# YuePanEdward/MULLS

Measured on NVIDIA H100. Metric: scan-pair registrations/sec (120k-pt 64-beam), higher is better.
Workload: dtype f32 geometry / f64 accumulation

## Files before the change

mulls_b200/csrc/device_types.cuh:

```cuda
#pragma once
#include <cstdint>
#include <cuda_runtime.h>

#include "../../include/mulls_b200/abi.h"
#include "search_core.cuh"

namespace mulls {

constexpr int kNumClasses = MULLS_NUM_CLASSES;
constexpr int kNumSegs = 2 * kNumClasses;
constexpr int kIterBlock = 128;
constexpr int kIngestBlock = 256;
constexpr int kTerms = 28;
constexpr int kMaxLevels = 12;
constexpr int kCoordBits = 12;
constexpr int kDedupMinSrc = 500;
constexpr unsigned kClaimFree = 0x7f7f7f7fu;
constexpr int kIterFlags = MULLS_MAX_TRACE_ITERS;

enum PairStatus : int { kRunning = 0, kNeedPosterior = 1, kDone = 2 };

struct ChunkDesc {
    uint32_t pair;
    uint32_t seg;
    uint32_t first;
};

struct PairConst {
    int max_iter;
    int used[kNumClasses];
    int w_balance, w_residual, w_dist, w_intensity;
    float z_xy_ratio;
    float win_pt2pt, win_pt2pl, win_pt2li;
    float thre_unit, thre_min, thre_rate;
    float conv_t, conv_r;
// ... 54 lines not shown
    int bb_src[6];
    int bb_tgt[6];
    uint64_t alg_bytes;
    int kl_keep[kNumSegs];
    uint32_t kl_rank[kNumSegs];
    uint64_t kl_prefix[kNumSegs];
    uint32_t kl_hist[kNumSegs][256];
};

struct LoopCtl {
    int it;
    int n_it_chunks;
    int n_pairs;
    int trace_on;
    int max_iter;
    unsigned solved;
    unsigned n_live[2];
    unsigned work[4];
};

struct DeviceArrays {
    const float4 *in_aos;
    uint64_t *keys_a, *keys_b;
    uint32_t *vals_a, *vals_b;
    float4 *tgt_pos, *tgt_nrm;
    float4 *src_pos[2], *src_nrm[2];
    int *src_prevj[2];
    float4 *src_cert[2];
    int *nn_idx;
    float *nn_d2;
    uint8_t *flags;
    int *corr_j;
    float *corr_w;
    unsigned *claim;
    HashEntry *hash;
    uint32_t hash_pool_entries;
    uint32_t *hash_used;
    uint32_t *blk_kept;
    double *partials;
    double *post_partials;
    PairConst *pc;
    PairState *ps;
    ChunkDesc *in_chunks;
    ChunkDesc *it_chunks;
    mulls_icp_trace *trace;
    int *xch_i32;
    double *xch_f64;
// ... 10 lines not shown
```

mulls_b200/csrc/kernels_ingest.cuh:

```cuda
#pragma once
#include "device_math.cuh"
#include "device_types.cuh"

namespace mulls {

template <bool kUndistort, bool kNormals>
__device__ __forceinline__ void load_input_point(const PairConst &pc, uint32_t seg, uint32_t local, float4 &pos, float4 &nrm) {
    const bool is_src = seg >= kNumClasses;
    const int cls = seg % kNumClasses;
    const bool undistort = kUndistort && is_src && pc.undistort && cls != MULLS_VERTEX;
    float x, y, z, intensity = 0.0f, curvature = 0.0f;
    float nx = 0.0f, ny = 0.0f, nz = 0.0f;
    const uint32_t fmt = pc.in_fmt[seg];
    if (fmt == 0u) {
        const float4 *in = pc.in_ptr[seg] + 3 * (size_t)local;
        const float4 a = in[0];
        x = a.x, y = a.y, z = a.z;
        if (kNormals) {
            const float4 b = in[1];
            const float4 c = in[2];
            nx = b.x, ny = b.y, nz = b.z;
            intensity = c.x, curvature = c.y;
        } else if (undistort) {
            curvature = reinterpret_cast<const float *>(in + 2)[1];
// ... 139 lines not shown
    for (int i = 0; i < 16; ++i) {
        ps.T_total[i] = pc.init[i];
        ps.T_inc[i] = (i % 5 == 0) ? 1.0 : 0.0;
    }
    for (int i = 0; i < 36; ++i) ps.cofactor[i] = ps.info[i] = (i % 7 == 0) ? 1.0 : 0.0;
    for (int i = 0; i < 6; ++i) ps.x[i] = 0.0;
    ps.sigma2 = 1.0;
    ps.thre = pc.thre_unit;
    ps.confidence = 1.0f;
    ps.status = kRunning;
    ps.code = 0;
    ps.iter = 0;
    ps.iters_entered = 0;
    ps.final_buf = 0;
    ps.alg_bytes = 0;
    if (pc.max_iter <= 0) {
        ps.status = kDone;
        const int left = atomicSub(A.running, 1) - 1;
        *A.h_running = left;
        __threadfence_system();
    }
}

template <bool kUndistort, bool kFiniteOnly = false>
__global__ void __launch_bounds__(kIngestBlock) k_make_keys(DeviceArrays A) {
    const ChunkDesc cd = A.in_chunks[blockIdx.x];
    const PairConst &pc = A.pc[cd.pair];
    PairState &ps = A.ps[cd.pair];
    const uint32_t seg = cd.seg;
    const uint32_t local = cd.first + threadIdx.x;
    const bool valid = local < pc.in_n[seg];
    bool inside = false;
    if (valid) {
        const size_t gi = (size_t)pc.in_off[seg] + local;
        float4 p, unused;
        load_input_point<kUndistort, false>(pc, seg, local, p, unused);
        const double *b = ps.ibb;
        inside = (double)p.x > b[0] && (double)p.x < b[3] && (double)p.y > b[1] && (double)p.y < b[4] &&
                 (double)p.z > b[2] && (double)p.z < b[5];
        if (kFiniteOnly) inside = inside && finite_xyz(p);
        uint64_t key = ~0ull;
        if (inside) {
            const int hi = (1 << kCoordBits) - 1;
            int cx = (int)floorf((p.x - ps.origin[0]) * ps.inv_h0);
            int cy = (int)floorf((p.y - ps.origin[1]) * ps.inv_h0);
            int cz = (int)floorf((p.z - ps.origin[2]) * ps.inv_h0);
            cx = min(max(cx, 0), hi);
            cy = min(max(cy, 0), hi);
            cz = min(max(cz, 0), hi);
            key = ((uint64_t)(cd.pair * kNumSegs + seg) << 36) | morton36((uint32_t)cx, (uint32_t)cy, (uint32_t)cz);
        }
        A.keys_a[gi] = key;
        A.vals_a[gi] = (uint32_t)gi;
    }
    const unsigned ballot = __ballot_sync(0xffffffffu, inside);
    if ((threadIdx.x & 31) == 0 && ballot) atomicAdd(&ps.seg_count[seg], (unsigned)__popc(ballot));
}

__device__ __forceinline__ uint64_t sample_key(uint32_t seed, uint32_t cloud_id, uint32_t index) {
    uint64_t z = (((uint64_t)seed << 40) ^ ((uint64_t)cloud_id << 32) ^ (uint64_t)index) + 0x9e3779b97f4a7c15ull;
    z = (z ^ (z >> 30)) * 0xbf58476d1ce4e5b9ull;
    z = (z ^ (z >> 27)) * 0x94d049bb133111ebull;
    return z ^ (z >> 31);
}

__global__ void k_keepless_plan(DeviceArrays A, int n_pairs) {
    const int p = blockIdx.x * blockDim.x + threadIdx.x;
    if (p >= n_pairs) return;
    const PairConst &pc = A.pc[p];
    PairState &ps = A.ps[p];
    for (int s = 0; s < kNumSegs; ++s) {
        ps.kl_keep[s] = -1;
        ps.kl_prefix[s] = 0;
        ps.kl_rank[s] = 0;
        for (int b = 0; b < 256; ++b) ps.kl_hist[s][b] = 0;
    }
    if (!pc.keep_less) return;
    const int S = kNumClasses;
    auto plan = [&](int seg, int keep) {
// ... 42 lines not shown
    PairState &ps = A.ps[p];
    for (int s = 0; s < kNumSegs; ++s) {
        if (ps.kl_keep[s] <= 0) continue;
        uint32_t cum = 0, rank = ps.kl_rank[s];
        int d = 0;
        for (; d < 256; ++d) {
            const uint32_t h = ps.kl_hist[s][d];
            if (cum + h >= rank) break;
            cum += h;
        }
        ps.kl_prefix[s] |= (uint64_t)d << (56 - 8 * pass);
        ps.kl_rank[s] = rank - cum;
        for (int b = 0; b < 256; ++b) ps.kl_hist[s][b] = 0;
    }
}

__global__ void __launch_bounds__(kIngestBlock) k_keepless_mark(DeviceArrays A) {
    const ChunkDesc cd = A.in_chunks[blockIdx.x];
    const PairConst &pc = A.pc[cd.pair];
    PairState &ps = A.ps[cd.pair];
    const uint32_t seg = cd.seg;
    const int keep = ps.kl_keep[seg];
    if (keep < 0) return;
    const uint32_t local = cd.first + threadIdx.x;
    bool drop = false;
    if (local < pc.in_n[seg]) {
        const size_t gi = (size_t)pc.in_off[seg] + local;
        if (A.keys_a[gi] != ~0ull) {
            drop = (keep == 0) || sample_key(pc.random_seed, seg, local) > ps.kl_prefix[seg];
            if (drop) A.keys_a[gi] = ~0ull;
        }
    }
    const unsigned b = __ballot_sync(0xffffffffu, drop);
    if ((threadIdx.x & 31) == 0 && b) atomicSub(&ps.seg_count[seg], (unsigned)__popc(b));
}

__global__ void k_seg_offsets(DeviceArrays A, int n_pairs) {
    __shared__ uint32_t carry;
    __shared__ uint32_t warp_sums[32];
    if (threadIdx.x == 0) carry = 0;
    __syncthreads();
    const int total = n_pairs * kNumSegs;
    for (int base = 0; base < total; base += blockDim.x) {
        const int i = base + threadIdx.x;
        uint32_t v = 0;
        if (i < total) v = A.ps[i / kNumSegs].seg_count[i % kNumSegs];
        uint32_t incl = v;
        for (int o = 1; o < 32; o <<= 1) {
            uint32_t t = __shfl_up_sync(0xffffffffu, incl, o);
            if ((threadIdx.x & 31) >= o) incl += t;
        }
        if ((threadIdx.x & 31) == 31) warp_sums[threadIdx.x >> 5] = incl;
        __syncthreads();
        if (threadIdx.x < 32) {
            uint32_t w = (threadIdx.x < (blockDim.x >> 5)) ? warp_sums[threadIdx.x] : 0;
            uint32_t wi = w;
            for (int o = 1; o < 32; o <<= 1) {
// ... 17 lines not shown
            ps.n_src[c] = (int)ps.seg_count[kNumClasses + c];
            ps.n_src_g[c] = ps.n_src[c];
            ps.n_corr[c] = 0;
            ps.n_corr_last[c] = 0;
        }
        int cnt = 0;
        if (pc.used[MULLS_PILLAR]) cnt += ps.n_src[MULLS_PILLAR];
        if (pc.used[MULLS_FACADE]) cnt += ps.n_src[MULLS_FACADE];
        if (pc.used[MULLS_BEAM]) cnt += ps.n_src[MULLS_BEAM];
        ps.source_feature_points_count = cnt;
    }
}

__device__ __forceinline__ int cell_top(const uint64_t *keys, uint32_t i, uint64_t kcur) {
    if (kcur == ~0ull || ((uint32_t)(kcur >> 36) % kNumSegs) >= kNumClasses) return -1;
    if (i == 0) return kMaxLevels - 1;
    const uint64_t kprev = keys[i - 1];
    if ((kprev >> 36) != (kcur >> 36)) return kMaxLevels - 1;
    const uint64_t diff = (kcur ^ kprev) & ((1ull << 36) - 1);
    if (diff == 0) return -1;
    return (63 - __clzll((long long)diff)) / 3;
}

template <bool kUndistort>
__global__ void __launch_bounds__(256) k_gather(DeviceArrays A, const uint64_t *keys, const uint32_t *vals, uint32_t n_total) {
    const uint32_t i = blockIdx.x * blockDim.x + threadIdx.x;
    const uint64_t key = i < n_total ? keys[i] : ~0ull;
    const uint32_t sg = (uint32_t)(key >> 36);
    const uint32_t pair = sg / kNumSegs, seg = sg % kNumSegs;
    const int top = cell_top(keys, i, key);
    const int cnt = top < 0 ? 0 : min(top, A.ps[pair].n_levels - 1) + 1;
    const bool is_tgt = key != ~0ull && seg < kNumClasses;
    const unsigned grp = __match_any_sync(0xffffffffu, is_tgt ? sg : 0xffffffffu);
    if (grp == 0xffffffffu) {
        const int tot = __reduce_add_sync(0xffffffffu, cnt);
        if ((threadIdx.x & 31) == 0 && tot > 0) atomicAdd(&A.ps[pair].hash_entries[seg], (unsigned)tot);
    } else if (cnt > 0) {
        atomicAdd(&A.ps[pair].hash_entries[seg], (unsigned)cnt);
    }
    if (key == ~0ull) return;
    const PairConst &pc = A.pc[pair];
    float4 pos, nrm;
    load_input_point<kUndistort, true>(pc, seg, vals[i] - pc.in_off[seg], pos, nrm);
    const uint32_t local = i - A.ps[pair].seg_start[seg];
    if (seg < kNumClasses) {
        const uint32_t d = pc.tgt_base[seg] + local;
        A.tgt_pos[d] = pos;
        A.tgt_nrm[d] = nrm;
    } else {
        const uint32_t d = pc.src_base[seg - kNumClasses] + local;
        if (pc.sharded) nrm.w = __int_as_float(__float_as_int(nrm.w) + (int)pc.src_index_base[seg - kNumClasses]);
        A.src_pos[0][d] = pos;
        A.src_nrm[0][d] = nrm;
    }
}

__device__ __forceinline__ void hash_insert(HashEntry *table, uint32_t hmask, uint32_t klo, uint32_t khi, uint32_t children,
                                            uint32_t start, uint32_t count) {
    uint32_t slot = cell_hash(klo, khi) & hmask;
    const unsigned long long packed = (unsigned long long)klo | ((unsigned long long)(khi | (children << 16)) << 32);
    while (true) {
        unsigned long long *kp = reinterpret_cast<unsigned long long *>(&table[slot]);
        if (atomicCAS(kp, 0ull, packed) == 0ull) {
            *reinterpret_cast<uint2 *>(&table[slot].start) = make_uint2(start, count);
            return;
        }
        slot = (slot + 1) & hmask;
    }
}

__device__ __forceinline__ uint32_t cell_end(const uint64_t *keys, uint32_t b, uint32_t hi, uint64_t p, int shift) {
    uint32_t in = b, out = hi, step = 1;
    while (in + step < hi) {
        if ((keys[in + step] >> shift) != p) {
            out = in + step;
            break;
        }
// ... 100 lines not shown
```

mulls_b200/csrc/mulls_b200.cu:

```cuda
#include <algorithm>
#include <atomic>
#include <cassert>
#include <memory>
#include <cmath>
#include <cstdio>
#include <chrono>
#include <cstring>
#include <string>
#include <vector>

#include <cub/device/device_radix_sort.cuh>
#include <cub/device/device_run_length_encode.cuh>
#include <cub/device/device_scan.cuh>
#include <cub/device/device_select.cuh>
#include <thrust/iterator/counting_iterator.h>

#include <dlfcn.h>
#include <mutex>

#include "device_types.cuh"
#include "host_pack.h"
#include "scan_io.h"
#include "kernels_ingest.cuh"
#include "kernels_iterate.cuh"
// ... 53 lines not shown
    return nccl_api().all_reduce(buf, buf, count, dtype == 0 ? 8 : 2, op == 0 ? 0 : 3, user, (cudaStream_t)stream);
}
}


struct mulls_map;

struct Scratch {
    void *p = nullptr;
    size_t bytes = 0;
    Scratch() = default;
    Scratch(const Scratch &) = delete;
    Scratch &operator=(const Scratch &) = delete;
    ~Scratch() { release(); }
    void release() {
        if (p) cudaFree(p);
        p = nullptr, bytes = 0;
    }
};

struct mulls_ctx {
    int device = 0;
    size_t max_pairs = 0, max_src = 0, max_tgt = 0;
    size_t cap_src = 0, cap_tgt = 0, cap_in = 0, cap_it_chunks = 0, cap_in_chunks = 0;
    cudaStream_t stream = nullptr;
    DeviceArrays A{};
    void *cub_temp = nullptr;
    size_t cub_temp_bytes = 0;
    mulls_icp_result *d_results = nullptr;
    mulls_icp_result *h_results = nullptr;
    uint32_t *h_flags = nullptr;
    int *h_running = nullptr;
    std::vector<cudaEvent_t> ev_done;
    mulls_icp_trace *d_trace = nullptr;
    std::vector<PairConst> h_pc;
    std::vector<ChunkDesc> h_in_chunks, h_it_chunks;
    size_t n_pairs = 0, n_in = 0, n_src_total = 0, n_tgt_total = 0;
    int max_iter_max = 0;
    bool uploaded = false;
    void *nccl_comm = nullptr;
    bool any_keep_less = false;
    bool grid_valid = false;
    int use_graph = 1;
    cudaGraph_t graph = nullptr;
    cudaGraphExec_t graph_exec = nullptr;
    int graph_key[2] = {-1, -1};
    uint64_t graph_body_launches = 0, graph_tail_launches = 0;
    LoopCtl *h_ctl = nullptr;
    int num_sms = 132;
    bool any_normal_shooting = false;
    bool any_undistort = false;
    int host_pack = 2;
    float4 *h_stage = nullptr;
    size_t h_stage_slots = 0;
    cudaEvent_t ev_begin = nullptr, ev_ingest = nullptr, ev_iter = nullptr, ev_end = nullptr, ev_h2d0 = nullptr;
    bool h2d_timed = false;
    float up_ms_pack = 0.f, up_ms_host = 0.f;
    std::vector<cudaEvent_t> ev_search;
    mulls_run_stats stats{};
// ... 163 lines not shown
    }
    mulls_ctx *ctx = new mulls_ctx();
    ctx->device = device;
    ctx->max_pairs = max_pairs;
    ctx->max_src = max_src_pts;
    ctx->max_tgt = max_tgt_pts;
    auto fail = [&](const char *what, cudaError_t err) -> mulls_ctx * {
        g_create_error = std::string("mulls_create: ") + what + ": " + cudaGetErrorString(err);
        mulls_destroy(ctx);
        return nullptr;
    };
    if ((e = cudaSetDevice(device)) != cudaSuccess) return fail("cudaSetDevice", e);
    if ((e = cudaStreamCreateWithFlags(&ctx->stream, cudaStreamNonBlocking)) != cudaSuccess) return fail("stream", e);
    const size_t cs = ctx->cap_src = max_pairs * max_src_pts;
    const size_t ct = ctx->cap_tgt = max_pairs * max_tgt_pts;
    const size_t cin = ctx->cap_in = cs + ct;
    if (cin >= (1ull << 31)) {
        g_create_error = "mulls_create: more than 2^31 points per context";
        mulls_destroy(ctx);
        return nullptr;
    }
    ctx->cap_it_chunks = ceil_div(cs, kIterBlock) + max_pairs * (kNumClasses + 1);
    ctx->cap_in_chunks = ceil_div(cin, kIngestBlock) + max_pairs * kNumSegs;
    DeviceArrays &A = ctx->A;
    float4 *in = nullptr;
#define ALLOC(ptr, n)                                                   \
    if ((e = dev_alloc(ctx, &(ptr), (n))) != cudaSuccess) return fail(#ptr, e)
    ALLOC(in, 3 * cin);
    A.in_aos = in;
    ALLOC(A.keys_a, cin);
    ALLOC(A.keys_b, cin);
    ALLOC(A.vals_a, cin);
    ALLOC(A.vals_b, cin);
    ALLOC(A.tgt_pos, ct + kScanOverrun);
    ALLOC(A.tgt_nrm, ct);
    for (int b = 0; b < 2; ++b) {
        ALLOC(A.src_pos[b], cs);
        ALLOC(A.src_nrm[b], cs);
        ALLOC(A.src_prevj[b], cs);
        ALLOC(A.src_cert[b], cs);
    }
    ALLOC(A.nn_idx, cs);
    ALLOC(A.nn_d2, cs);
    ALLOC(A.flags, cs);
    ALLOC(A.corr_j, cs);
    ALLOC(A.corr_w, cs);
    ALLOC(A.claim, ct);
    {
        size_t pool = 12 * ct + 64 * max_pairs * kNumClasses;
        if (pool >= (1ull << 32)) pool = (1ull << 32) - 1;
        A.hash_pool_entries = (uint32_t)pool;
        ALLOC(A.hash, pool);
    }
    ALLOC(A.hash_used, 3);
    ALLOC(A.ctl, 1);
    ALLOC(A.blk_kept, ctx->cap_it_chunks);
// ... 13 lines not shown
    ALLOC(ctx->d_results, max_pairs + ceil_div(max_pairs * sizeof(uint64_t), sizeof(mulls_icp_result)) + 1);
    ALLOC(ctx->d_trace, max_pairs);
    ALLOC(A.running, 1);
    ALLOC(A.xch_i32, 32);
    ALLOC(A.xch_f64, kNumClasses * kTerms + 8);
#undef ALLOC
    if ((e = cudaHostAlloc((void **)&ctx->h_running, (1 + kIterFlags) * sizeof(int), cudaHostAllocMapped)) != cudaSuccess)
        return fail("mapped flag", e);
    {
        int *dptr = nullptr;
        if ((e = cudaHostGetDevicePointer((void **)&dptr, ctx->h_running, 0)) != cudaSuccess) return fail("mapped flag", e);
        A.h_running = dptr;
        A.h_running_iter = dptr + 1;
    }
    ctx->ev_done.resize(MULLS_MAX_TRACE_ITERS);
    for (auto &ev : ctx->ev_done) cudaEventCreateWithFlags(&ev, cudaEventDisableTiming);
    A.trace = ctx->d_trace;
    if ((e = cudaMallocHost((void **)&ctx->h_results, max_pairs * (sizeof(mulls_icp_result) + sizeof(uint64_t)))) != cudaSuccess)
        return fail("pinned results", e);
    if ((e = cudaMallocHost((void **)&ctx->h_flags, 4 * sizeof(uint32_t))) != cudaSuccess) return fail("pinned flags", e);
    if ((e = cudaMallocHost((void **)&ctx->h_ctl, sizeof(LoopCtl))) != cudaSuccess) return fail("pinned control block", e);
    {
        size_t bytes = 0;
        cub::DeviceRadixSort::SortPairs(nullptr, bytes, A.keys_a, A.keys_b, A.vals_a, A.vals_b, (int)cin, 0, 64,
                                        ctx->stream);
        ctx->cub_temp_bytes = bytes;
        if ((e = cudaMalloc(&ctx->cub_temp, std::max<size_t>(bytes, 16))) != cudaSuccess) return fail("cub temp", e);
    }
    cudaEventCreate(&ctx->ev_begin);
    cudaEventCreate(&ctx->ev_ingest);
    cudaEventCreate(&ctx->ev_iter);
    cudaEventCreate(&ctx->ev_end);
    cudaEventCreate(&ctx->ev_h2d0);
    ctx->ev_search.resize(2 * MULLS_MAX_TRACE_ITERS);
    for (auto &ev : ctx->ev_search) cudaEventCreate(&ev);
    if ((e = cudaMemsetAsync(A.ps, 0, max_pairs * sizeof(PairState), ctx->stream)) != cudaSuccess) return fail("memset", e);
    if ((e = cudaStreamSynchronize(ctx->stream)) != cudaSuccess) return fail("sync", e);
    return ctx;
}

int mulls_set_tunable(mulls_ctx *ctx, const char *name, int value) {
    if (!ctx || !name) return MULLS_E_ARG;
    if (ctx->twin) {
        const int rc = mulls_set_tunable(ctx->twin, name, value);
        if (rc != MULLS_OK) return rc;
    }
    std::string n(name);
    if (n == "use_graph") ctx->use_graph = value;
    else if (n == "host_pack") ctx->host_pack = value;
    else if (n == "pack_threads") PackPool::get().ensure_workers(value);
    else return MULLS_E_ARG;
    return MULLS_OK;
}

int mulls_pack_rows(const float *aos48, size_t n, int format, float *out) {
    if ((n > 0 && (!aos48 || !out)) || (format != kFmtPacked28 && format != kFmtPacked32) || ((uintptr_t)out % 16) != 0)
        return MULLS_E_ARG;
    pack_rows(aos48, 0, n, format, out, out + 4 * n);
    _mm_sfence();
// ... 134 lines not shown
    for (int i = 0; i < 16; ++i) pc.init[i] = init[i];
    for (int i = 0; i < 6; ++i) pc.tbound[i] = P.target_bound[i];
    return MULLS_OK;
}

static int upload_impl(mulls_ctx *ctx, size_t n_pairs, const mulls_cloud_view *tgt, const mulls_cloud_view *src,
                       const mulls_icp_params *params, const double *init_guess, const uint32_t *src_index_base,
                       const uint32_t *src_global_n, bool resident = true, bool tgt_on_device = false) {
    if (!ctx || !tgt || !src || !params || !init_guess || n_pairs == 0) return MULLS_E_ARG;
    ctx->tree_map = nullptr;
    ctx->grid_valid = false;
    if (n_pairs > ctx->max_pairs) {
        ctx->err = "more pairs than the context was created for";
        return MULLS_E_CAPACITY;
    }
    CK(cudaSetDevice(ctx->device));
    ctx->uploaded = false;
    const double t_up0 = wall_ms();
    ctx->h2d_timed = false;
    ctx->up_ms_pack = 0.f;
    ctx->h_pc.assign(n_pairs, PairConst());
    ctx->h_in_chunks.clear();
    ctx->h_it_chunks.clear();
    size_t in_off = 0, s_off = 0, t_off = 0;
    int max_iter_max = 0;
    bool any_keep_less = false, any_shoot = false, any_undistort = false;
    for (size_t p = 0; p < n_pairs; ++p) {
        PairConst &pc = ctx->h_pc[p];
        int rc = build_pair_const(ctx, params[p], init_guess + 16 * p, pc);
        if (rc != MULLS_OK) return rc;
        max_iter_max = std::max(max_iter_max, pc.max_iter);
        any_keep_less = any_keep_less || pc.keep_less;
        any_shoot = any_shoot || pc.normal_shooting;
        any_undistort = any_undistort || pc.undistort;
        size_t ns = 0, nt = 0;
        for (int c = 0; c < kNumClasses; ++c) {
            nt += tgt[p * kNumClasses + c].n;
            ns += src[p * kNumClasses + c].n;
        }
        if (ns > ctx->max_src || nt > ctx->max_tgt) {
            ctx->err = "pair exceeds max_src_pts / max_tgt_pts of the context";
            return MULLS_E_CAPACITY;
        }
        for (int s = 0; s < kNumSegs; ++s) {
            const mulls_cloud_view &v = (s < kNumClasses) ? tgt[p * kNumClasses + s] : src[p * kNumClasses + (s - kNumClasses)];
            if (v.n > 0 && !v.aos48) return MULLS_E_ARG;
            pc.in_off[s] = (uint32_t)in_off;
            pc.in_n[s] = (uint32_t)v.n;
            for (size_t f = 0; f < v.n; f += kIngestBlock)
                ctx->h_in_chunks.push_back(ChunkDesc{(uint32_t)p, (uint32_t)s, (uint32_t)f});
            in_off += v.n;
        }
        pc.chunk_begin = (uint32_t)ctx->h_it_chunks.size();
        for (int c = 0; c < kNumClasses; ++c) {
            pc.tgt_base[c] = (uint32_t)t_off;
            pc.src_base[c] = (uint32_t)s_off;
            t_off += tgt[p * kNumClasses + c].n;
            const size_t n = src[p * kNumClasses + c].n;
            s_off += n;
            pc.class_chunk_begin[c] = (uint32_t)ctx->h_it_chunks.size();
            const size_t n_eff = (c == 0 && n == 0) ? 1 : n;
            for (size_t f = 0; f < n_eff; f += kIterBlock) ctx->h_it_chunks.push_back(ChunkDesc{(uint32_t)p, (uint32_t)c, (uint32_t)f});
            pc.src_index_base[c] = src_index_base ? src_index_base[c] : 0;
            pc.src_global_n[c] = src_global_n ? src_global_n[c] : (uint32_t)n;
        }
        pc.class_chunk_begin[kNumClasses] = (uint32_t)ctx->h_it_chunks.size();
        pc.chunk_end = (uint32_t)ctx->h_it_chunks.size();
        pc.sharded = src_index_base ? 1 : 0;
    }
    if (ctx->h_in_chunks.size() > ctx->cap_in_chunks || ctx->h_it_chunks.size() > ctx->cap_it_chunks) {
        ctx->err = "internal: chunk table capacity";
        return MULLS_E_CAPACITY;
    }
    size_t host_points = 0;
    for (size_t p = 0; p < n_pairs; ++p)
        for (int s = 0; s < kNumSegs; ++s)
            if (!(tgt_on_device && s < kNumClasses)) host_points += ctx->h_pc[p].in_n[s];
    const size_t kPackMinPoints = 1u << 18;
    bool tables_sent = false;
    const bool pack = ctx->host_pack == 1 || (ctx->host_pack == 2 && host_points >= kPackMinPoints);
    if (pack) {
        if (!ctx->h_stage) {
            const size_t slots = 2 * ctx->cap_in + 4 * kNumSegs * ctx->max_pairs;
            CK(cudaHostAlloc((void **)&ctx->h_stage, slots * sizeof(float4), cudaHostAllocDefault));
            ctx->h_stage_slots = slots;
        }
        CK(cudaStreamSynchronize(ctx->stream));
        PackPool &pool = PackPool::get();
        pool.ensure_workers(0);
        std::unique_ptr<std::atomic<int>[]> pending(new std::atomic<int>[n_pairs]);
        std::vector<size_t> slot_begin(n_pairs + 1, 0);
        std::vector<PackJob> jobs;
        const size_t kJobPts = 16384;
// ... 16 lines not shown
                float *pos = reinterpret_cast<float *>(ctx->h_stage + slot);
                float *nrm = reinterpret_cast<float *>(ctx->h_stage + slot + v.n);
                for (size_t f = 0; f < v.n; f += kJobPts) {
                    jobs.push_back(PackJob{v.aos48, pos, nrm, f, std::min(kJobPts, v.n - f), fmt, &pending[p]});
                    ++n_jobs;
                }
                slot += packed_slots(v.n, fmt);
            }
            pending[p].store(n_jobs, std::memory_order_relaxed);
        }
        slot_begin[n_pairs] = slot;
        if (slot > ctx->h_stage_slots || slot > 3 * ctx->cap_in) {
            ctx->err = "internal: packed staging capacity";
            return MULLS_E_CAPACITY;
        }
        pool.submit(jobs);
        cudaError_t ce = cudaMemcpyAsync(ctx->A.pc, ctx->h_pc.data(), n_pairs * sizeof(PairConst), cudaMemcpyHostToDevice, ctx->stream);
        if (ce == cudaSuccess && !ctx->h_in_chunks.empty())
            ce = cudaMemcpyAsync(ctx->A.in_chunks, ctx->h_in_chunks.data(), ctx->h_in_chunks.size() * sizeof(ChunkDesc),
                                 cudaMemcpyHostToDevice, ctx->stream);
        if (ce == cudaSuccess && !ctx->h_it_chunks.empty())
            ce = cudaMemcpyAsync(ctx->A.it_chunks, ctx->h_it_chunks.data(), ctx->h_it_chunks.size() * sizeof(ChunkDesc),
                                 cudaMemcpyHostToDevice, ctx->stream);
        tables_sent = true;
        if (ce == cudaSuccess && cudaEventRecord(ctx->ev_h2d0, ctx->stream) == cudaSuccess) ctx->h2d_timed = true;
        const double t_pack0 = wall_ms();
        for (size_t p = 0; p < n_pairs; ++p) {
            pool.help_until_done(pending[p]);
            if (p + 1 == n_pairs) ctx->up_ms_pack = (float)(wall_ms() - t_pack0);
            const size_t b = slot_begin[p], e = slot_begin[p + 1];
            if (e > b && ce == cudaSuccess)
                ce = cudaMemcpyAsync((void *)(ctx->A.in_aos + b), ctx->h_stage + b, (e - b) * sizeof(float4), cudaMemcpyHostToDevice,
                                     ctx->stream);
        }
        CK(ce);
    } else {
    if (cudaEventRecord(ctx->ev_h2d0, ctx->stream) == cudaSuccess) ctx->h2d_timed = true;
    for (size_t p = 0; p < n_pairs; ++p) {
        PairConst &pc = ctx->h_pc[p];
        for (int s = 0; s < kNumSegs; ++s) {
            const mulls_cloud_view &v = (s < kNumClasses) ? tgt[p * kNumClasses + s] : src[p * kNumClasses + (s - kNumClasses)];
            pc.in_ptr[s] = ctx->A.in_aos + 3 * (size_t)pc.in_off[s];
            pc.in_fmt[s] = kFmtRows48;
            if (v.n == 0) continue;
            if (tgt_on_device && s < kNumClasses) {
                pc.in_ptr[s] = (const float4 *)v.aos48;
                continue;
            }
            CK(cudaMemcpyAsync((void *)(ctx->A.in_aos + 3 * (size_t)pc.in_off[s]), v.aos48, v.n * 48, cudaMemcpyHostToDevice,
                               ctx->stream));
        }
    }
    }
    if (!tables_sent) {
        CK(cudaMemcpyAsync(ctx->A.pc, ctx->h_pc.data(), n_pairs * sizeof(PairConst), cudaMemcpyHostToDevice, ctx->stream));
        if (!ctx->h_in_chunks.empty())
            CK(cudaMemcpyAsync(ctx->A.in_chunks, ctx->h_in_chunks.data(), ctx->h_in_chunks.size() * sizeof(ChunkDesc),
                               cudaMemcpyHostToDevice, ctx->stream));
        if (!ctx->h_it_chunks.empty())
            CK(cudaMemcpyAsync(ctx->A.it_chunks, ctx->h_it_chunks.data(), ctx->h_it_chunks.size() * sizeof(ChunkDesc),
                               cudaMemcpyHostToDevice, ctx->stream));
    }
    if (resident) CK(cudaStreamSynchronize(ctx->stream));
    ctx->n_pairs = n_pairs;
    ctx->n_in = in_off;
    ctx->n_src_total = s_off;
    ctx->n_tgt_total = t_off;
    ctx->max_iter_max = max_iter_max;
    ctx->any_keep_less = any_keep_less;
    ctx->any_normal_shooting = any_shoot;
    ctx->any_undistort = any_undistort;
    ctx->uploaded = true;
    ctx->up_ms_host = (float)(wall_ms() - t_up0);
    return MULLS_OK;
}

static int exchange(mulls_ctx *ctx, mulls_allreduce_fn hook, void *user, void *buf, size_t count, int dtype, int op) {
    if (hook(user, buf, count, dtype, op, (void *)ctx->stream) == 0) return MULLS_OK;
    ctx->err = "all-reduce callback failed";
    return MULLS_E_COMM;
}

static int launch_ingest(mulls_ctx *ctx, DeviceArrays &A, bool trace, uint64_t &launches, mulls_allreduce_fn hook = nullptr,
                         void *user = nullptr, bool finite_only = false) {
    cudaStream_t st = ctx->stream;
    const int np = (int)ctx->n_pairs;
    const uint32_t n_in = (uint32_t)ctx->n_in;
    if (trace) CK(cudaMemsetAsync(ctx->d_trace, 0, np * sizeof(mulls_icp_trace), st));
    CK(cudaMemsetAsync(A.claim, 0x7f, std::max<size_t>(ctx->n_tgt_total, 1) * sizeof(unsigned), st));
    k_state_init<<<(unsigned)ceil_div(np, 128), 128, 0, st>>>(A, np);
    ++launches;
    const unsigned n_inc = (unsigned)ctx->h_in_chunks.size();
    if (n_inc) {
        if (ctx->any_undistort) k_ingest_bbox<true><<<n_inc, kIngestBlock, 0, st>>>(A);
        else if (finite_only) k_ingest_bbox<false, true><<<n_inc, kIngestBlock, 0, st>>>(A);
        else k_ingest_bbox<false><<<n_inc, kIngestBlock, 0, st>>>(A);
        ++launches;
    }
    if (hook) {
        k_shard_pack_setup<<<1, 1, 0, st>>>(A, 0);
        if (const int rc = exchange(ctx, hook, user, A.xch_i32, 6, 1, 1); rc != MULLS_OK) return rc;
        k_shard_pack_setup<<<1, 1, 0, st>>>(A, 1);
        launches += 2;
    }
    k_pair_setup<<<(unsigned)ceil_div(np, 128), 128, 0, st>>>(A, np);
    ++launches;
    if (n_inc) {
        if (ctx->any_undistort) k_make_keys<true><<<n_inc, kIngestBlock, 0, st>>>(A);
        else if (finite_only) k_make_keys<false, true><<<n_inc, kIngestBlock, 0, st>>>(A);
        else k_make_keys<false><<<n_inc, kIngestBlock, 0, st>>>(A);
        ++launches;
        if (ctx->any_keep_less) {
            const unsigned pb = (unsigned)ceil_div(np, 64);
            k_keepless_plan<<<pb, 64, 0, st>>>(A, np);
            for (int pass = 0; pass < 8; ++pass) {
                k_keepless_hist<<<n_inc, kIngestBlock, 0, st>>>(A, pass);
                k_keepless_step<<<pb, 64, 0, st>>>(A, np, pass);
            }
            k_keepless_mark<<<n_inc, kIngestBlock, 0, st>>>(A);
            launches += 18;
        }
        int seg_bits = 1;
        while ((1ull << seg_bits) <= (uint64_t)np * kNumSegs) ++seg_bits;
        size_t bytes = ctx->cub_temp_bytes;
        CK(cub::DeviceRadixSort::SortPairs(ctx->cub_temp, bytes, A.keys_a, A.keys_b, A.vals_a, A.vals_b, (int)n_in, 0,
                                           36 + seg_bits, st));
    }
    k_seg_offsets<<<1, 256, 0, st>>>(A, np);
    ++launches;
    if (hook) {
        k_shard_pack_setup<<<1, 1, 0, st>>>(A, 2);
        if (const int rc = exchange(ctx, hook, user, A.xch_i32, kNumClasses, 1, 0); rc != MULLS_OK) return rc;
        k_shard_pack_setup<<<1, 1, 0, st>>>(A, 3);
        launches += 2;
    }
    if (n_in) {
        const unsigned nb = (unsigned)ceil_div(n_in, 256);
        if (ctx->any_undistort) k_gather<true><<<nb, 256, 0, st>>>(A, A.keys_b, A.vals_b, n_in);
        else k_gather<false><<<nb, 256, 0, st>>>(A, A.keys_b, A.vals_b, n_in);
        k_hash_layout<<<1, 32, 0, st>>>(A, np);
        k_hash_clear<<<1184, 256, 0, st>>>(A);
        k_hash_build<<<nb, 256, 0, st>>>(A, A.keys_b, n_in);
        launches += 4;
    } else {
        k_hash_layout<<<1, 32, 0, st>>>(A, np);
        ++launches;
    }
    return MULLS_OK;
}

static unsigned chunk_bucket(const mulls_ctx *ctx) {
    unsigned b = 1;
    while (b < (unsigned)ctx->h_it_chunks.size()) b <<= 1;
    return b;
}
static unsigned resident_grid(const mulls_ctx *ctx, int blocks_per_sm, unsigned chunks_per_block = 1) {
    return std::min((unsigned)(ctx->num_sms * blocks_per_sm), (chunk_bucket(ctx) + chunks_per_block - 1) / chunks_per_block);
}
constexpr int kShootBlocksPerSm = 8;
constexpr int kPollPause = 64;

static int enqueue_iteration(mulls_ctx *ctx, int it, mulls_allreduce_fn hook, void *user, unsigned long long handle,
                             uint64_t &launches) {
    cudaStream_t st = ctx->stream;
    const DeviceArrays &A = ctx->A;
    const bool recording = it < 0;
// ... 2407 lines not shown
```

Measured before the change: 6578.

## Replace CUB pair sort with custom segmented onepass radix sort fused with gather

```diff
diff --git a/mulls_b200/csrc/device_types.cuh b/mulls_b200/csrc/device_types.cuh
--- a/mulls_b200/csrc/device_types.cuh
+++ b/mulls_b200/csrc/device_types.cuh
@@ -11,6 +11,11 @@
 constexpr int kNumSegs = 2 * kNumClasses;
 constexpr int kIterBlock = 128;
 constexpr int kIngestBlock = 256;
+constexpr int kSortDigitBits = 9;
+constexpr int kSortBins = 1 << kSortDigitBits;
+constexpr int kSortPasses = 4;
+constexpr int kSortItems = 16;
+constexpr int kSortTile = kIngestBlock * kSortItems;
 constexpr int kTerms = 28;
 constexpr int kMaxLevels = 12;
 constexpr int kCoordBits = 12;
@@ -111,7 +116,10 @@
 struct DeviceArrays {
     const float4 *in_aos;
     uint64_t *keys_a, *keys_b;
-    uint32_t *vals_a, *vals_b;
+    ChunkDesc *sort_tiles;
+    uint32_t *digit_hist;
+    uint64_t *sort_status;
+    uint32_t *sort_ctr;
     float4 *tgt_pos, *tgt_nrm;
     float4 *src_pos[2], *src_nrm[2];
     int *src_prevj[2];
diff --git a/mulls_b200/csrc/kernels_ingest.cuh b/mulls_b200/csrc/kernels_ingest.cuh
--- a/mulls_b200/csrc/kernels_ingest.cuh
+++ b/mulls_b200/csrc/kernels_ingest.cuh
@@ -185,39 +185,64 @@
     }
 }
 
+__device__ __forceinline__ uint64_t cell_morton(const PairState &ps, const float4 &p) {
+    const int hi = (1 << kCoordBits) - 1;
+    const int cx = (int)floorf((p.x - ps.origin[0]) * ps.inv_h0);
+    const int cy = (int)floorf((p.y - ps.origin[1]) * ps.inv_h0);
+    const int cz = (int)floorf((p.z - ps.origin[2]) * ps.inv_h0);
+    return morton36((uint32_t)min(max(cx, 0), hi), (uint32_t)min(max(cy, 0), hi), (uint32_t)min(max(cz, 0), hi));
+}
+
+__device__ __forceinline__ uint32_t *digit_hist_of(const DeviceArrays &A, uint32_t pair, uint32_t seg) {
+    return A.digit_hist + (size_t)(pair * kNumSegs + seg) * (kSortPasses * kSortBins);
+}
+__device__ __forceinline__ void digit_hist_add(uint32_t (*s_hist)[kSortBins], bool on, uint64_t m) {
+    const unsigned lt = (1u << (threadIdx.x & 31)) - 1u;
+#pragma unroll
+    for (int d = 0; d < kSortPasses; ++d) {
+        const uint32_t b = on ? (uint32_t)(m >> (kSortDigitBits * d)) & (kSortBins - 1) : kSortBins;
+        const unsigned peers = __match_any_sync(0xffffffffu, b);
+        if (on && (peers & lt) == 0) atomicAdd(&s_hist[d][b], (unsigned)__popc(peers));
+    }
+}
+__device__ __forceinline__ void digit_hist_flush(uint32_t (*s_hist)[kSortBins], uint32_t *g, bool subtract) {
+    for (int i = threadIdx.x; i < kSortPasses * kSortBins; i += blockDim.x) {
+        const uint32_t c = s_hist[i / kSortBins][i % kSortBins];
+        if (c) atomicAdd(&g[i], subtract ? 0u - c : c);
+    }
+}
+
 template <bool kUndistort, bool kFiniteOnly = false>
 __global__ void __launch_bounds__(kIngestBlock) k_make_keys(DeviceArrays A) {
-    const ChunkDesc cd = A.in_chunks[blockIdx.x];
-    const PairConst &pc = A.pc[cd.pair];
-    PairState &ps = A.ps[cd.pair];
-    const uint32_t seg = cd.seg;
-    const uint32_t local = cd.first + threadIdx.x;
-    const bool valid = local < pc.in_n[seg];
-    bool inside = false;
-    if (valid) {
-        const size_t gi = (size_t)pc.in_off[seg] + local;
-        float4 p, unused;
-        load_input_point<kUndistort, false>(pc, seg, local, p, unused);
-        const double *b = ps.ibb;
-        inside = (double)p.x > b[0] && (double)p.x < b[3] && (double)p.y > b[1] && (double)p.y < b[4] &&
-                 (double)p.z > b[2] && (double)p.z < b[5];
-        if (kFiniteOnly) inside = inside && finite_xyz(p);
-        uint64_t key = ~0ull;
-        if (inside) {
-            const int hi = (1 << kCoordBits) - 1;
-            int cx = (int)floorf((p.x - ps.origin[0]) * ps.inv_h0);
-            int cy = (int)floorf((p.y - ps.origin[1]) * ps.inv_h0);
-            int cz = (int)floorf((p.z - ps.origin[2]) * ps.inv_h0);
-            cx = min(max(cx, 0), hi);
-            cy = min(max(cy, 0), hi);
-            cz = min(max(cz, 0), hi);
-            key = ((uint64_t)(cd.pair * kNumSegs + seg) << 36) | morton36((uint32_t)cx, (uint32_t)cy, (uint32_t)cz);
-        }
-        A.keys_a[gi] = key;
-        A.vals_a[gi] = (uint32_t)gi;
-    }
-    const unsigned ballot = __ballot_sync(0xffffffffu, inside);
-    if ((threadIdx.x & 31) == 0 && ballot) atomicAdd(&ps.seg_count[seg], (unsigned)__popc(ballot));
+    const ChunkDesc td = A.sort_tiles[blockIdx.x];
+    const PairConst &pc = A.pc[td.pair];
+    PairState &ps = A.ps[td.pair];
+    const uint32_t seg = td.seg;
+    __shared__ uint32_t s_hist[kSortPasses][kSortBins];
+    for (int i = threadIdx.x; i < kSortPasses * kSortBins; i += kIngestBlock) s_hist[i / kSortBins][i % kSortBins] = 0;
+    __syncthreads();
+    unsigned kept = 0;
+#pragma unroll 1
+    for (int k = 0; k < kSortItems; ++k) {
+        const uint32_t local = td.first + k * kIngestBlock + threadIdx.x;
+        bool inside = false;
+        uint64_t m = 0;
+        if (local < pc.in_n[seg]) {
+            float4 p, unused;
+            load_input_point<kUndistort, false>(pc, seg, local, p, unused);
+            const double *b = ps.ibb;
+            inside = (double)p.x > b[0] && (double)p.x < b[3] && (double)p.y > b[1] && (double)p.y < b[4] &&
+                     (double)p.z > b[2] && (double)p.z < b[5];
+            if (kFiniteOnly) inside = inside && finite_xyz(p);
+            if (inside) m = cell_morton(ps, p);
+            A.keys_a[(size_t)pc.in_off[seg] + local] = inside ? m : ~0ull;
+        }
+        digit_hist_add(s_hist, inside, m);
+        kept += (unsigned)__popc(__ballot_sync(0xffffffffu, inside));
+    }
+    if ((threadIdx.x & 31) == 0 && kept) atomicAdd(&ps.seg_count[seg], kept);
+    __syncthreads();
+    digit_hist_flush(s_hist, digit_hist_of(A, td.pair, seg), false);
 }
 
 __device__ __forceinline__ uint64_t sample_key(uint32_t seed, uint32_t cloud_id, uint32_t index) {
@@ -306,17 +331,64 @@
     const uint32_t seg = cd.seg;
     const int keep = ps.kl_keep[seg];
     if (keep < 0) return;
+    __shared__ uint32_t s_hist[kSortPasses][kSortBins];
+    for (int i = threadIdx.x; i < kSortPasses * kSortBins; i += kIngestBlock) s_hist[i / kSortBins][i % kSortBins] = 0;
+    __syncthreads();
     const uint32_t local = cd.first + threadIdx.x;
     bool drop = false;
+    uint64_t m = 0;
     if (local < pc.in_n[seg]) {
         const size_t gi = (size_t)pc.in_off[seg] + local;
-        if (A.keys_a[gi] != ~0ull) {
+        m = A.keys_a[gi];
+        if (m != ~0ull) {
             drop = (keep == 0) || sample_key(pc.random_seed, seg, local) > ps.kl_prefix[seg];
             if (drop) A.keys_a[gi] = ~0ull;
         }
     }
+    digit_hist_add(s_hist, drop, m);
     const unsigned b = __ballot_sync(0xffffffffu, drop);
     if ((threadIdx.x & 31) == 0 && b) atomicSub(&ps.seg_count[seg], (unsigned)__popc(b));
+    __syncthreads();
+    digit_hist_flush(s_hist, digit_hist_of(A, cd.pair, seg), true);
+}
+
+template <int kThreads>
+__device__ __forceinline__ uint32_t block_exclusive_scan(uint32_t v, uint32_t *s_warp, uint32_t &total) {
+    const int lane = threadIdx.x & 31, w = threadIdx.x >> 5;
+    uint32_t incl = v;
+#pragma unroll
+    for (int o = 1; o < 32; o <<= 1) {
+        const uint32_t t = __shfl_up_sync(0xffffffffu, incl, o);
+        if (lane >= o) incl += t;
+    }
+    if (lane == 31) s_warp[w] = incl;
+    __syncthreads();
+    if (w == 0) {
+        const uint32_t x = lane < kThreads / 32 ? s_warp[lane] : 0u;
+        uint32_t xi = x;
+#pragma unroll
+        for (int o = 1; o < 32; o <<= 1) {
+            const uint32_t t = __shfl_up_sync(0xffffffffu, xi, o);
+            if (lane >= o) xi += t;
+        }
+        if (lane < kThreads / 32) s_warp[lane] = xi - x;
+        if (lane == 31) s_warp[32] = xi;
+    }
+    __syncthreads();
+    total = s_warp[32];
+    const uint32_t r = s_warp[w] + incl - v;
+    __syncthreads();
+    return r;
+}
+
+__global__ void __launch_bounds__(kSortBins) k_digit_scan(DeviceArrays A) {
+    __shared__ uint32_t s_warp[33];
+    uint32_t *h = A.digit_hist + (size_t)blockIdx.x * (kSortPasses * kSortBins);
+    for (int d = 0; d < kSortPasses; ++d) {
+        uint32_t total;
+        const uint32_t v = h[d * kSortBins + threadIdx.x];
+        h[d * kSortBins + threadIdx.x] = block_exclusive_scan<kSortBins>(v, s_warp, total);
+    }
 }
 
 __global__ void k_seg_offsets(DeviceArrays A, int n_pairs) {
@@ -380,8 +452,159 @@
     return (63 - __clzll((long long)diff)) / 3;
 }
 
-template <bool kUndistort>
-__global__ void __launch_bounds__(256) k_gather(DeviceArrays A, const uint64_t *keys, const uint32_t *vals, uint32_t n_total) {
+struct SortSmem {
+    union {
+        uint32_t warp_bin[kIngestBlock / 32][kSortBins];
+        struct {
+            uint64_t item[kSortTile];
+            uint16_t bin[kSortTile];
+        } stage;
+    } u;
+    uint32_t tile_start[kSortBins];
+    uint32_t out_base[kSortBins];
+    uint32_t warp_sum[33];
+    uint32_t tile, n_tile;
+};
+
+template <int kPass>
+__device__ __forceinline__ uint32_t sort_digit(uint64_t e) {
+    return (uint32_t)(kPass == 0 ? e : e >> 31) & (kSortBins - 1);
+}
+
+template <int kPass, bool kUndistort>
+__global__ void __launch_bounds__(kIngestBlock, 3) k_sort_pass(DeviceArrays A, const uint64_t *in, uint64_t *out, int n_pairs,
+                                                            uint32_t epoch) {
+    constexpr bool kLast = kPass == kSortPasses - 1;
+    __shared__ SortSmem s;
+    if (threadIdx.x == 0) s.tile = atomicAdd(&A.sort_ctr[kPass], 1u);
+    for (int i = threadIdx.x; i < (kIngestBlock / 32) * kSortBins; i += kIngestBlock) (&s.u.warp_bin[0][0])[i] = 0;
+    __syncthreads();
+    const uint32_t t = s.tile;
+    const ChunkDesc td = A.sort_tiles[t];
+    const PairConst &pc = A.pc[td.pair];
+    const PairState &ps = A.ps[td.pair];
+    const uint32_t seg = td.seg;
+    const uint32_t n = kPass == 0 ? pc.in_n[seg] : ps.seg_count[seg];
+    if (kLast) {
+        const PairState &pl = A.ps[n_pairs - 1];
+        const uint32_t kept = pl.seg_start[kNumSegs - 1] + pl.seg_count[kNumSegs - 1];
+        const uint32_t tail = kept + (pc.in_off[seg] - ps.seg_start[seg]) - n;
+        for (uint32_t i = max(td.first, n) + threadIdx.x; i < min(td.first + kSortTile, pc.in_n[seg]); i += kIngestBlock)
+            out[tail + i] = ~0ull;
+    }
+    if (td.first >= n) return;
+    const uint64_t *src = in + pc.in_off[seg];
+    const int w = threadIdx.x >> 5, lane = threadIdx.x & 31;
+    const unsigned lt = (1u << lane) - 1u;
+    uint64_t item[kSortItems];
+    uint32_t rb[kSortItems];
+#pragma unroll
+    for (int j = 0; j < kSortItems; ++j) {
+        const uint32_t idx = td.first + (w * kSortItems + j) * 32 + lane;
+        uint64_t e = idx < n ? src[idx] : ~0ull;
+        const bool valid = e != ~0ull;
+        const uint32_t b = valid ? sort_digit<kPass>(e) : kSortBins;
+        const unsigned peers = __match_any_sync(0xffffffffu, b);
+        uint32_t r = 0;
+        if (valid) r = s.u.warp_bin[w][b] + (uint32_t)__popc(peers & lt);
+        __syncwarp();
+        if (valid && (peers & lt) == 0) s.u.warp_bin[w][b] += (uint32_t)__popc(peers);
+        __syncwarp();
+        if (kPass == 0) e = ((e >> kSortDigitBits) << 31) | idx;
+        else if (!kLast) e = ((e >> (31 + kSortDigitBits)) << 31) | (e & 0x7fffffffu);
+        else e &= 0x7fffffffu;
+        item[j] = e;
+        rb[j] = r | (b << 16);
+    }
+    __syncthreads();
+    uint32_t cnt[2];
+#pragma unroll
+    for (int q = 0; q < 2; ++q) {
+        const int b = 2 * threadIdx.x + q;
+        uint32_t run = 0;
+#pragma unroll
+        for (int v = 0; v < kIngestBlock / 32; ++v) {
+            const uint32_t c = s.u.warp_bin[v][b];
+            s.u.warp_bin[v][b] = run;
+            run += c;
+        }
+        cnt[q] = run;
+    }
+    uint32_t n_tile;
+    const uint32_t ex = block_exclusive_scan<kIngestBlock>(cnt[0] + cnt[1], s.warp_sum, n_tile);
+    s.tile_start[2 * threadIdx.x] = ex;
+    s.tile_start[2 * threadIdx.x + 1] = ex + cnt[0];
+    volatile uint64_t *status = A.sort_status;
+    const uint64_t agg = (uint64_t)(2u * epoch) << 32, inc = (uint64_t)(2u * epoch + 1u) << 32;
+#pragma unroll
+    for (int q = 0; q < 2; ++q) status[(size_t)t * kSortBins + 2 * threadIdx.x + q] = (td.first == 0 ? inc : agg) | cnt[q];
+    const uint32_t *dig = digit_hist_of(A, td.pair, seg) + kPass * kSortBins;
+    const uint32_t base = kLast ? ps.seg_start[seg] : pc.in_off[seg];
+#pragma unroll
+    for (int q = 0; q < 2; ++q) {
+        const int b = 2 * threadIdx.x + q;
+        uint32_t prefix = 0;
+        if (td.first != 0) {
+            for (uint32_t k = t - 1;; --k) {
+                uint64_t v;
+                do v = status[(size_t)k * kSortBins + b];
+                while ((uint32_t)(v >> 32) < 2u * epoch);
+                prefix += (uint32_t)v;
+                if ((uint32_t)(v >> 32) & 1u) break;
+            }
+            status[(size_t)t * kSortBins + b] = inc | (prefix + cnt[q]);
+        }
+        s.out_base[b] = base + dig[b] + prefix - s.tile_start[b];
+    }
+    __syncthreads();
+    uint32_t pos[kSortItems];
+#pragma unroll
+    for (int j = 0; j < kSortItems; ++j) {
+        const uint32_t b = rb[j] >> 16;
+        pos[j] = b < kSortBins ? s.tile_start[b] + s.u.warp_bin[w][b] + (rb[j] & 0xffffu) : 0u;
+    }
+    __syncthreads();
+#pragma unroll
+    for (int j = 0; j < kSortItems; ++j) {
+        const uint32_t b = rb[j] >> 16;
+        if (b < kSortBins) {
+            s.u.stage.item[pos[j]] = item[j];
+            s.u.stage.bin[pos[j]] = (uint16_t)b;
+        }
+    }
+    __syncthreads();
+    if (!kLast) {
+        for (uint32_t p = threadIdx.x; p < n_tile; p += kIngestBlock) out[s.out_base[s.u.stage.bin[p]] + p] = s.u.stage.item[p];
+        return;
+    }
+    const uint32_t sg = td.pair * kNumSegs + seg;
+    constexpr int kGather = 4;
+    const uint32_t dst_base = seg < kNumClasses ? pc.tgt_base[seg] : pc.src_base[seg - kNumClasses];
+    const int index_shift = (seg >= kNumClasses && pc.sharded) ? (int)pc.src_index_base[seg - kNumClasses] : 0;
+    float4 *dst_pos = seg < kNumClasses ? A.tgt_pos : A.src_pos[0];
+    float4 *dst_nrm = seg < kNumClasses ? A.tgt_nrm : A.src_nrm[0];
+    for (uint32_t p0 = threadIdx.x; p0 < n_tile; p0 += kGather * kIngestBlock) {
+        float4 pt[kGather], nrm[kGather];
+#pragma unroll
+        for (int g = 0; g < kGather; ++g) {
+            const uint32_t p = p0 + g * kIngestBlock;
+            if (p < n_tile) load_input_point<kUndistort, true>(pc, seg, (uint32_t)s.u.stage.item[p], pt[g], nrm[g]);
+        }
+#pragma unroll
+        for (int g = 0; g < kGather; ++g) {
+            const uint32_t p = p0 + g * kIngestBlock;
+            if (p >= n_tile) break;
+            const uint32_t i = s.out_base[s.u.stage.bin[p]] + p;
+            out[i] = ((uint64_t)sg << 36) | cell_morton(ps, pt[g]);
+            const uint32_t d = dst_base + (i - ps.seg_start[seg]);
+            nrm[g].w = __int_as_float(__float_as_int(nrm[g].w) + index_shift);
+            dst_pos[d] = pt[g];
+            dst_nrm[d] = nrm[g];
+        }
+    }
+}
+
+__global__ void __launch_bounds__(256) k_cell_count(DeviceArrays A, const uint64_t *keys, uint32_t n_total) {
     const uint32_t i = blockIdx.x * blockDim.x + threadIdx.x;
     const uint64_t key = i < n_total ? keys[i] : ~0ull;
     const uint32_t sg = (uint32_t)(key >> 36);
@@ -396,21 +619,18 @@
     } else if (cnt > 0) {
         atomicAdd(&A.ps[pair].hash_entries[seg], (unsigned)cnt);
     }
-    if (key == ~0ull) return;
-    const PairConst &pc = A.pc[pair];
-    float4 pos, nrm;
-    load_input_point<kUndistort, true>(pc, seg, vals[i] - pc.in_off[seg], pos, nrm);
-    const uint32_t local = i - A.ps[pair].seg_start[seg];
-    if (seg < kNumClasses) {
-        const uint32_t d = pc.tgt_base[seg] + local;
-        A.tgt_pos[d] = pos;
-        A.tgt_nrm[d] = nrm;
-    } else {
-        const uint32_t d = pc.src_base[seg - kNumClasses] + local;
-        if (pc.sharded) nrm.w = __int_as_float(__float_as_int(nrm.w) + (int)pc.src_index_base[seg - kNumClasses]);
-        A.src_pos[0][d] = pos;
-        A.src_nrm[0][d] = nrm;
-    }
+}
+
+inline void enqueue_sort_pass(const DeviceArrays &A, cudaStream_t st, int pass, unsigned n_tiles, int n_pairs, bool undistort,
+                              uint32_t &epoch) {
+    const uint64_t *in = (pass & 1) ? A.keys_b : A.keys_a;
+    uint64_t *out = (pass & 1) ? A.keys_a : A.keys_b;
+    ++epoch;
+    if (pass == 0) k_sort_pass<0, false><<<n_tiles, kIngestBlock, 0, st>>>(A, in, out, n_pairs, epoch);
+    else if (pass == 1) k_sort_pass<1, false><<<n_tiles, kIngestBlock, 0, st>>>(A, in, out, n_pairs, epoch);
+    else if (pass == 2) k_sort_pass<2, false><<<n_tiles, kIngestBlock, 0, st>>>(A, in, out, n_pairs, epoch);
+    else if (undistort) k_sort_pass<3, true><<<n_tiles, kIngestBlock, 0, st>>>(A, in, out, n_pairs, epoch);
+    else k_sort_pass<3, false><<<n_tiles, kIngestBlock, 0, st>>>(A, in, out, n_pairs, epoch);
 }
 
 __device__ __forceinline__ void hash_insert(HashEntry *table, uint32_t hmask, uint32_t klo, uint32_t khi, uint32_t children,
diff --git a/mulls_b200/csrc/mulls_b200.cu b/mulls_b200/csrc/mulls_b200.cu
--- a/mulls_b200/csrc/mulls_b200.cu
+++ b/mulls_b200/csrc/mulls_b200.cu
@@ -99,7 +99,7 @@
 struct mulls_ctx {
     int device = 0;
     size_t max_pairs = 0, max_src = 0, max_tgt = 0;
-    size_t cap_src = 0, cap_tgt = 0, cap_in = 0, cap_it_chunks = 0, cap_in_chunks = 0;
+    size_t cap_src = 0, cap_tgt = 0, cap_in = 0, cap_it_chunks = 0, cap_in_chunks = 0, cap_sort_tiles = 0;
     cudaStream_t stream = nullptr;
     DeviceArrays A{};
     void *cub_temp = nullptr;
@@ -111,7 +111,8 @@
     std::vector<cudaEvent_t> ev_done;
     mulls_icp_trace *d_trace = nullptr;
     std::vector<PairConst> h_pc;
-    std::vector<ChunkDesc> h_in_chunks, h_it_chunks;
+    std::vector<ChunkDesc> h_in_chunks, h_it_chunks, h_sort_tiles;
+    uint32_t sort_epoch = 0;
     size_t n_pairs = 0, n_in = 0, n_src_total = 0, n_tgt_total = 0;
     int max_iter_max = 0;
     bool uploaded = false;
@@ -321,6 +322,7 @@
     }
     ctx->cap_it_chunks = ceil_div(cs, kIterBlock) + max_pairs * (kNumClasses + 1);
     ctx->cap_in_chunks = ceil_div(cin, kIngestBlock) + max_pairs * kNumSegs;
+    ctx->cap_sort_tiles = ceil_div(cin, kSortTile) + max_pairs * kNumSegs;
     DeviceArrays &A = ctx->A;
     float4 *in = nullptr;
 #define ALLOC(ptr, n)                                                   \
@@ -329,8 +331,10 @@
     A.in_aos = in;
     ALLOC(A.keys_a, cin);
     ALLOC(A.keys_b, cin);
-    ALLOC(A.vals_a, cin);
-    ALLOC(A.vals_b, cin);
+    ALLOC(A.sort_tiles, ctx->cap_sort_tiles);
+    ALLOC(A.digit_hist, max_pairs * kNumSegs * kSortPasses * kSortBins);
+    ALLOC(A.sort_status, ctx->cap_sort_tiles * kSortBins);
+    ALLOC(A.sort_ctr, kSortPasses);
     ALLOC(A.tgt_pos, ct + kScanOverrun);
     ALLOC(A.tgt_nrm, ct);
     for (int b = 0; b < 2; ++b) {
@@ -390,8 +394,7 @@
     if ((e = cudaMallocHost((void **)&ctx->h_ctl, sizeof(LoopCtl))) != cudaSuccess) return fail("pinned control block", e);
     {
         size_t bytes = 0;
-        cub::DeviceRadixSort::SortPairs(nullptr, bytes, A.keys_a, A.keys_b, A.vals_a, A.vals_b, (int)cin, 0, 64,
-                                        ctx->stream);
+        cub::DeviceRadixSort::SortKeys(nullptr, bytes, A.keys_a, A.keys_b, (int)cin, 0, 64, ctx->stream);
         ctx->cub_temp_bytes = bytes;
         if ((e = cudaMalloc(&ctx->cub_temp, std::max<size_t>(bytes, 16))) != cudaSuccess) return fail("cub temp", e);
     }
@@ -403,6 +406,8 @@
     ctx->ev_search.resize(2 * MULLS_MAX_TRACE_ITERS);
     for (auto &ev : ctx->ev_search) cudaEventCreate(&ev);
     if ((e = cudaMemsetAsync(A.ps, 0, max_pairs * sizeof(PairState), ctx->stream)) != cudaSuccess) return fail("memset", e);
+    if ((e = cudaMemsetAsync(A.sort_status, 0, ctx->cap_sort_tiles * kSortBins * sizeof(uint64_t), ctx->stream)) != cudaSuccess)
+        return fail("memset", e);
     if ((e = cudaStreamSynchronize(ctx->stream)) != cudaSuccess) return fail("sync", e);
     return ctx;
 }
@@ -583,6 +588,7 @@
     ctx->h_pc.assign(n_pairs, PairConst());
     ctx->h_in_chunks.clear();
     ctx->h_it_chunks.clear();
+    ctx->h_sort_tiles.clear();
     size_t in_off = 0, s_off = 0, t_off = 0;
     int max_iter_max = 0;
     bool any_keep_less = false, any_shoot = false, any_undistort = false;
@@ -610,6 +616,8 @@
             pc.in_n[s] = (uint32_t)v.n;
             for (size_t f = 0; f < v.n; f += kIngestBlock)
                 ctx->h_in_chunks.push_back(ChunkDesc{(uint32_t)p, (uint32_t)s, (uint32_t)f});
+            for (size_t f = 0; f < v.n; f += kSortTile)
+                ctx->h_sort_tiles.push_back(ChunkDesc{(uint32_t)p, (uint32_t)s, (uint32_t)f});
             in_off += v.n;
         }
         pc.chunk_begin = (uint32_t)ctx->h_it_chunks.size();
@@ -629,7 +637,8 @@
         pc.chunk_end = (uint32_t)ctx->h_it_chunks.size();
         pc.sharded = src_index_base ? 1 : 0;
     }
-    if (ctx->h_in_chunks.size() > ctx->cap_in_chunks || ctx->h_it_chunks.size() > ctx->cap_it_chunks) {
+    if (ctx->h_in_chunks.size() > ctx->cap_in_chunks || ctx->h_it_chunks.size() > ctx->cap_it_chunks ||
+        ctx->h_sort_tiles.size() > ctx->cap_sort_tiles) {
         ctx->err = "internal: chunk table capacity";
         return MULLS_E_CAPACITY;
     }
@@ -692,6 +701,9 @@
         if (ce == cudaSuccess && !ctx->h_it_chunks.empty())
             ce = cudaMemcpyAsync(ctx->A.it_chunks, ctx->h_it_chunks.data(), ctx->h_it_chunks.size() * sizeof(ChunkDesc),
                                  cudaMemcpyHostToDevice, ctx->stream);
+        if (ce == cudaSuccess && !ctx->h_sort_tiles.empty())
+            ce = cudaMemcpyAsync(ctx->A.sort_tiles, ctx->h_sort_tiles.data(), ctx->h_sort_tiles.size() * sizeof(ChunkDesc),
+                                 cudaMemcpyHostToDevice, ctx->stream);
         tables_sent = true;
         if (ce == cudaSuccess && cudaEventRecord(ctx->ev_h2d0, ctx->stream) == cudaSuccess) ctx->h2d_timed = true;
         const double t_pack0 = wall_ms();
@@ -730,6 +742,9 @@
         if (!ctx->h_it_chunks.empty())
             CK(cudaMemcpyAsync(ctx->A.it_chunks, ctx->h_it_chunks.data(), ctx->h_it_chunks.size() * sizeof(ChunkDesc),
                                cudaMemcpyHostToDevice, ctx->stream));
+        if (!ctx->h_sort_tiles.empty())
+            CK(cudaMemcpyAsync(ctx->A.sort_tiles, ctx->h_sort_tiles.data(), ctx->h_sort_tiles.size() * sizeof(ChunkDesc),
+                               cudaMemcpyHostToDevice, ctx->stream));
     }
     if (resident) CK(cudaStreamSynchronize(ctx->stream));
     ctx->n_pairs = n_pairs;
@@ -775,10 +790,13 @@
     }
     k_pair_setup<<<(unsigned)ceil_div(np, 128), 128, 0, st>>>(A, np);
     ++launches;
+    const unsigned n_tiles = (unsigned)ctx->h_sort_tiles.size();
     if (n_inc) {
-        if (ctx->any_undistort) k_make_keys<true><<<n_inc, kIngestBlock, 0, st>>>(A);
-        else if (finite_only) k_make_keys<false, true><<<n_inc, kIngestBlock, 0, st>>>(A);
-        else k_make_keys<false><<<n_inc, kIngestBlock, 0, st>>>(A);
+        CK(cudaMemsetAsync(A.digit_hist, 0, (size_t)np * kNumSegs * kSortPasses * kSortBins * sizeof(uint32_t), st));
+        CK(cudaMemsetAsync(A.sort_ctr, 0, kSortPasses * sizeof(uint32_t), st));
+        if (ctx->any_undistort) k_make_keys<true><<<n_tiles, kIngestBlock, 0, st>>>(A);
+        else if (finite_only) k_make_keys<false, true><<<n_tiles, kIngestBlock, 0, st>>>(A);
+        else k_make_keys<false><<<n_tiles, kIngestBlock, 0, st>>>(A);
         ++launches;
         if (ctx->any_keep_less) {
             const unsigned pb = (unsigned)ceil_div(np, 64);
@@ -790,11 +808,10 @@
             k_keepless_mark<<<n_inc, kIngestBlock, 0, st>>>(A);
             launches += 18;
         }
-        int seg_bits = 1;
-        while ((1ull << seg_bits) <= (uint64_t)np * kNumSegs) ++seg_bits;
-        size_t bytes = ctx->cub_temp_bytes;
-        CK(cub::DeviceRadixSort::SortPairs(ctx->cub_temp, bytes, A.keys_a, A.keys_b, A.vals_a, A.vals_b, (int)n_in, 0,
-                                           36 + seg_bits, st));
+        k_digit_scan<<<(unsigned)(np * kNumSegs), kSortBins, 0, st>>>(A);
+        for (int pass = 0; pass < kSortPasses - 1; ++pass)
+            enqueue_sort_pass(A, st, pass, n_tiles, np, ctx->any_undistort, ctx->sort_epoch);
+        launches += kSortPasses;
     }
     k_seg_offsets<<<1, 256, 0, st>>>(A, np);
     ++launches;
@@ -806,12 +823,12 @@
     }
     if (n_in) {
         const unsigned nb = (unsigned)ceil_div(n_in, 256);
-        if (ctx->any_undistort) k_gather<true><<<nb, 256, 0, st>>>(A, A.keys_b, A.vals_b, n_in);
-        else k_gather<false><<<nb, 256, 0, st>>>(A, A.keys_b, A.vals_b, n_in);
+        enqueue_sort_pass(A, st, kSortPasses - 1, n_tiles, np, ctx->any_undistort, ctx->sort_epoch);
+        k_cell_count<<<nb, 256, 0, st>>>(A, A.keys_a, n_in);
         k_hash_layout<<<1, 32, 0, st>>>(A, np);
         k_hash_clear<<<1184, 256, 0, st>>>(A);
-        k_hash_build<<<nb, 256, 0, st>>>(A, A.keys_b, n_in);
-        launches += 4;
+        k_hash_build<<<nb, 256, 0, st>>>(A, A.keys_a, n_in);
+        launches += 5;
     } else {
         k_hash_layout<<<1, 32, 0, st>>>(A, np);
         ++launches;
```

Result: faster. 6809, median of 6 (+3.5%).
